# googleinterns/multimodal-long-transformer-2021

Hardware: AMD Instinct MI355X
Metric: train-step samples/sec + attention TFLOPS, 4096-tok seq (higher is better)
Workload: dtype bf16; 1 GPU; BASELINE config 3: BERT-base dims, S=4096 (2+63^2 patches+125 text), radius 64 + 8 global tokens, bf16, per-GPU batch 4; step=train_step, per_gpu_batch=4, global_batch=4, seq_len=4096, parallelism=dp1, ranks_seen=1, params=111009852, optimizer=AdamW (fused flat step, bf16 shadow weights) + polynomial lr, clip 1.0, grad_allreduce=none (1 GPU), grad_reduce=mean, step_launch=HIP graph replay (recorded after 3 eager steps)

## Files before the change

### multimodal-long-transformer-2021_amd/csrc/embed.hip

```cpp
#include "../../include/mmt_attn.h"
#include "../../include/mmt_layer.h"

#include "layer_common.h"
#include "mmt_err.h"

namespace mmt {

constexpr int kEmbedCut = 32;
constexpr int kEmbedBlocks = 1024;

struct EmbedParams {
  long rows;
  int S, H, vocab, seg_vocab, patch_start, n_patch;
  float eps, inv_keep;
  uint32_t thresh16, seed_lo, seed_hi;
  const unsigned long long* epoch;
  const int *word_ids, *seg_ids, *order, *sorted_ids;
  const float *word_table, *seg_table, *pos_table, *gamma, *beta, *patch_bias;
  const void* patch;
  void* out;
  float *mean_out, *rstd_out;
  const void* dout;
  const float *mean, *rstd;
  float* dword_table;
  float* part;
  float* pieces;
  void* dpatch;
  int nblocks;
  const int *starts, *slots;
  int n_ex, pos_rows;
  const int *image_entry, *text_entry, *prefix_ids, *text_ids, *text_len;
  int n_images, n_texts;
  int* valid_len_out;
};

struct PackedPos { int local, e, pj; bool has_patch; };
__device__ __forceinline__ PackedPos packed_pos(const EmbedParams& p, long row, int s) {
  PackedPos o;
  const int st = min(max(p.starts[row], 0), p.S - 1);
  o.local = min(max(s - st, 0), p.S - 1);
  o.e = p.slots ? p.slots[row] : -1;
  o.pj = o.local - p.patch_start;
// ... 78 lines not shown
      load_param(p.beta + c * 8, bt);
#pragma unroll
      for (int i = 0; i < 8; ++i) {
        float w = (v[j][i] - mean) * rstd * g[i] + bt[i];
        if (p.thresh16) w = layer_drop_bits16(layer_drop_row(sd.lo, sd.hi, row), (uint32_t)(c * 8 + i)) >= p.thresh16 ? w * p.inv_keep : 0.f;
        y[i] = w;
      }
      if (sg_ok) {
        load_param(p.seg_table + (long)sg * p.H + c * 8, t);
#pragma unroll
        for (int i = 0; i < 8; ++i) y[i] += t[i];
      }
      if (p.pos_table) {
        load_param(p.pos_table + (long)ps * p.H + c * 8, t);
#pragma unroll
        for (int i = 0; i < 8; ++i) y[i] += t[i];
      }
      if (has_patch) {
        Chunk<T>::load(reinterpret_cast<const T*>(p.patch) + ((long)pe * p.n_patch + pj) * p.H + c * 8, t);
#pragma unroll
        for (int i = 0; i < 8; ++i) y[i] += t[i];
        if (p.patch_bias) {
          load_param(p.patch_bias + c * 8, t);
#pragma unroll
          for (int i = 0; i < 8; ++i) y[i] += t[i];
        }
      }
      Chunk<T>::store(reinterpret_cast<T*>(p.out) + off, y);
    }
  }
}

template <typename T, int NCH, bool PK = false>
__global__ __launch_bounds__(256) void embed_bwd_kernel(const EmbedParams p) {
  const SeedPair sd = effective_seed(p.seed_lo, p.seed_hi, p.epoch);
  __shared__ float red[4][64 * NCH * 8];
  const int lane = threadIdx.x & 63, wave = threadIdx.x >> 6;
  const int nch = p.H >> 3;
  const float invH = 1.f / (float)p.H;
  float acc_g[NCH][8], acc_bt[NCH][8], gam[NCH][8];
#pragma unroll
  for (int j = 0; j < NCH; ++j) {
#pragma unroll
    for (int i = 0; i < 8; ++i) { acc_g[j][i] = 0.f; acc_bt[j][i] = 0.f; gam[j][i] = 0.f; }
    if (lane + 64 * j < nch) load_param(p.gamma + (lane + 64 * j) * 8, gam[j]);
  }
  for (long pos = (long)blockIdx.x * 4 + wave; pos < p.rows; pos += (long)gridDim.x * 4) {
    const int id = p.sorted_ids[pos];
    const bool first = pos == 0 || p.sorted_ids[pos - 1] != id;
    if (!first && (pos % kEmbedCut) != 0) continue;
    const long cut = (pos / kEmbedCut + 1) * kEmbedCut;
    const long lim = cut < p.rows ? cut : p.rows;
    const bool id_ok = (unsigned)id < (unsigned)p.vocab;
    float xw[NCH][8], acc[NCH][8];
#pragma unroll
    for (int j = 0; j < NCH; ++j) {
#pragma unroll
      for (int i = 0; i < 8; ++i) { xw[j][i] = 0.f; acc[j][i] = 0.f; }
      if (id_ok && lane + 64 * j < nch) load_param(p.word_table + (long)id * p.H + (lane + 64 * j) * 8, xw[j]);
    }
    int n_rows, rowv = 0;
    {
      const long me = pos + (lane & 31);
      const bool in_piece = me < lim && p.sorted_ids[me] == id;
      if (me < lim) rowv = p.order[me];
      const unsigned long long mism = ~__ballot(in_piece) & 0xFFFFFFFFull;
      n_rows = mism ? __builtin_ctzll(mism) : 32;
    }
    const long e = pos + n_rows;
    const int row0 = __builtin_amdgcn_readfirstlane(rowv);
    const float mean = p.mean[row0], rstd = p.rstd[row0];
    float tsum[NCH][8];
#pragma unroll
    for (int j = 0; j < NCH; ++j)
#pragma unroll
      for (int i = 0; i < 8; ++i) tsum[j][i] = 0.f;
    for (int k0 = 0; k0 < n_rows; k0 += 4) {
      float t[4][NCH][8];
      int rows4[4];
#pragma unroll
      for (int u = 0; u < 4; ++u) {
        const int k = min(k0 + u, n_rows - 1);
        rows4[u] = __builtin_amdgcn_readlane(rowv, k);
#pragma unroll
        for (int j = 0; j < NCH; ++j) {
          const int c = lane + 64 * j;
#pragma unroll
          for (int i = 0; i < 8; ++i) t[u][j][i] = 0.f;
          if (c < nch && k0 + u < n_rows) Chunk<T>::load(reinterpret_cast<const T*>(p.dout) + (long)rows4[u] * p.H + c * 8, t[u][j]);
        }
      }
#pragma unroll
// ... 22 lines not shown
          }
        }
      }
    }
    {
      float xh[NCH][8];
      float s1 = 0.f, s2 = 0.f;
#pragma unroll
      for (int j = 0; j < NCH; ++j)
#pragma unroll
        for (int i = 0; i < 8; ++i) {
          const bool live = lane + 64 * j < nch;
          xh[j][i] = live ? (xw[j][i] - mean) * rstd : 0.f;
          const float dyh = tsum[j][i] * gam[j][i];
          s1 += dyh;
          s2 += dyh * xh[j][i];
          acc_g[j][i] += tsum[j][i] * xh[j][i];
          acc_bt[j][i] += tsum[j][i];
        }
      const float c1 = wave_sum(s1) * invH, c2 = wave_sum(s2) * invH;
#pragma unroll
      for (int j = 0; j < NCH; ++j)
#pragma unroll
        for (int i = 0; i < 8; ++i) acc[j][i] = rstd * (tsum[j][i] * gam[j][i] - c1 - xh[j][i] * c2);
    }
    const bool run_ends = e >= p.rows || p.sorted_ids[e] != id;
    const bool whole = first && run_ends;
    if (!id_ok) continue;
#pragma unroll
    for (int j = 0; j < NCH; ++j) {
      const int c = lane + 64 * j;
      if (c >= nch) continue;
      if (whole) {
        float* dst = p.dword_table + (long)id * p.H + c * 8;
        float cur[8];
        load_param(dst, cur);
#pragma unroll
        for (int i = 0; i < 8; ++i) cur[i] += acc[j][i];
        Chunk<float>::store(dst, cur);
      } else {
        Chunk<float>::store(p.pieces + pos * p.H + c * 8, acc[j]);
      }
    }
  }
  int set = 0;
  auto flush = [&](float (&a)[NCH][8]) {
    __syncthreads();
#pragma unroll
    for (int j = 0; j < NCH; ++j)
#pragma unroll
      for (int i = 0; i < 8; ++i) red[wave][(lane + 64 * j) * 8 + i] = a[j][i];
    __syncthreads();
    for (int col = threadIdx.x; col < p.H; col += 256)
      p.part[((long)blockIdx.x * 2 + set) * p.H + col] = (red[0][col] + red[1][col]) + (red[2][col] + red[3][col]);
    ++set;
  };
  flush(acc_g);
  flush(acc_bt);
}

template <int NCH>
__global__ __launch_bounds__(256) void embed_bwd_runs_kernel(const EmbedParams p) {
  const int lane = threadIdx.x & 63, wave = threadIdx.x >> 6;
  const int nch = p.H >> 3;
  for (long pos = (long)blockIdx.x * 4 + wave; pos < p.rows; pos += (long)gridDim.x * 4) {
    const int id = p.sorted_ids[pos];
    const bool first = pos == 0 || p.sorted_ids[pos - 1] != id;
    const long cut = (pos / kEmbedCut + 1) * kEmbedCut;
    if (!first || cut >= p.rows || p.sorted_ids[cut] != id || (unsigned)id >= (unsigned)p.vocab) continue;
    float acc[NCH][8];
#pragma unroll
    for (int j = 0; j < NCH; ++j) {
#pragma unroll
      for (int i = 0; i < 8; ++i) acc[j][i] = 0.f;
      if (lane + 64 * j < nch) load_param(p.pieces + pos * p.H + (lane + 64 * j) * 8, acc[j]);
    }
    for (long q = cut; q < p.rows && p.sorted_ids[q] == id; q += kEmbedCut) {
#pragma unroll
      for (int j = 0; j < NCH; ++j)
        if (lane + 64 * j < nch) {
          float t[8];
          load_param(p.pieces + q * p.H + (lane + 64 * j) * 8, t);
#pragma unroll
          for (int i = 0; i < 8; ++i) acc[j][i] += t[i];
        }
    }
#pragma unroll
    for (int j = 0; j < NCH; ++j) {
      const int c = lane + 64 * j;
      if (c >= nch) continue;
      float* dst = p.dword_table + (long)id * p.H + c * 8;
      float cur[8];
      load_param(dst, cur);
#pragma unroll
      for (int i = 0; i < 8; ++i) cur[i] += acc[j][i];
      Chunk<float>::store(dst, cur);
    }
  }
// ... 87 lines not shown
int mmt_embed_fwd_pairs(const mmt_embed_desc* d, const int32_t* image_entry, const int32_t* text_entry,
                        const int32_t* prefix_ids, const int32_t* text_ids, const int32_t* text_len, int32_t n_images,
                        int32_t n_texts, const float* word_table, const float* seg_table, const float* pos_table,
                        const float* gamma, const float* beta, const void* patch_proj, const float* patch_bias,
                        void* out, int32_t* valid_len_out, void* stream) {
  if (int rc = check_embed(d)) return rc;
  if (d->dropout_p != 0.f) return mmt::fail(MMT_E_UNSUPPORTED, "mmt_embed_fwd_pairs: forward for prediction only, dropout_p must be 0");
  if (!image_entry || !text_entry || !prefix_ids || !text_ids || !text_len || !word_table || !seg_table || !gamma || !beta ||
      !out || !valid_len_out)
    return mmt::fail(MMT_E_INVALID, "mmt_embed_fwd_pairs: NULL argument");
  if ((long)d->patch_start + d->n_patch >= d->S)
    return mmt::fail(MMT_E_INVALID, "mmt_embed_fwd_pairs: the image part [0, %d) leaves no room for text in S=%d",
                     d->patch_start + d->n_patch, d->S);
  if (d->n_patch > 0 && !patch_proj) return mmt::fail(MMT_E_INVALID, "mmt_embed_fwd_pairs: n_patch > 0 but patch_proj is NULL");
  mmt::EmbedParams p; fill_embed(p, d);
  p.word_table = word_table; p.seg_table = seg_table; p.pos_table = pos_table; p.gamma = gamma; p.beta = beta;
  p.patch = d->n_patch > 0 ? patch_proj : nullptr; p.patch_bias = patch_bias; p.out = out;
  p.image_entry = image_entry; p.text_entry = text_entry; p.prefix_ids = prefix_ids; p.text_ids = text_ids;
  p.text_len = text_len; p.n_images = n_images > 0 ? n_images : 0; p.n_texts = n_texts > 0 ? n_texts : 0;
  p.valid_len_out = valid_len_out;
  const int blocks = embed_blocks(d), nchl = ((d->H >> 3) + 63) / 64;
  hipStream_t st = (hipStream_t)stream;
#define MMT_EP(T, N) hipLaunchKernelGGL((mmt::embed_fwd_kernel<T, N, false, true>), dim3(blocks), dim3(256), 0, st, p)
#define MMT_EPN(T) do { if (nchl <= 1) MMT_EP(T, 1); else if (nchl <= 2) MMT_EP(T, 2); else MMT_EP(T, 4); } while (0)
  if (d->dtype == MMT_BF16) MMT_EPN(__bf16); else MMT_EPN(float);
#undef MMT_EPN
#undef MMT_EP
  hipError_t e = hipGetLastError();
  return e == hipSuccess ? MMT_OK : mmt::fail(MMT_E_LAUNCH, "mmt_embed_fwd_pairs: %s", hipGetErrorString(e));
}

size_t mmt_embed_workspace_bytes(const mmt_embed_desc* d) {
  if (!d || d->H <= 0 || d->rows <= 0) return 0;
  return ((size_t)mmt::kEmbedBlocks * 2 * d->H + (size_t)d->rows * d->H) * sizeof(float);
}

static int embed_bwd_any(const mmt_embed_desc* d, const void* dout, const int32_t* sorted_ids, const int32_t* order,
                  const float* word_table, const float* gamma, const float* mean, const float* rstd,
                  float* dword_table, float* dgamma, float* dbeta, void* dpatch, void* ws, size_t ws_bytes,
                  const int32_t* starts, const int32_t* slots, int n_ex, void* stream) {
  if (int rc = check_embed(d)) return rc;
  if (!dout || !sorted_ids || !order || !word_table || !gamma || !mean || !rstd || !dword_table || !dgamma || !dbeta)
    return mmt::fail(MMT_E_INVALID, "mmt_embed_bwd: NULL argument");
  if (!ws || ws_bytes < mmt_embed_workspace_bytes(d)) return mmt::fail(MMT_E_WORKSPACE, "mmt_embed_bwd: workspace too small");
  mmt::EmbedParams p; fill_embed(p, d);
  p.dout = dout; p.sorted_ids = sorted_ids; p.order = order; p.word_table = word_table; p.gamma = gamma;
  p.mean = mean; p.rstd = rstd; p.dword_table = dword_table; p.dpatch = d->n_patch > 0 ? dpatch : nullptr;
  p.part = (float*)ws; p.pieces = p.part + (size_t)mmt::kEmbedBlocks * 2 * d->H;
  p.nblocks = embed_blocks(d);
  p.starts = starts; p.slots = slots; p.n_ex = n_ex;
  const int nchl = ((d->H >> 3) + 63) / 64;
  hipStream_t st = (hipStream_t)stream;
#define MMT_EB(T, N, PK) hipLaunchKernelGGL((mmt::embed_bwd_kernel<T, N, PK>), dim3(p.nblocks), dim3(256), 0, st, p)
#define MMT_EBN(T, PK) do { if (nchl <= 1) MMT_EB(T, 1, PK); else if (nchl <= 2) MMT_EB(T, 2, PK); else MMT_EB(T, 4, PK); } while (0)
  if (starts) { if (d->dtype == MMT_BF16) MMT_EBN(__bf16, true); else MMT_EBN(float, true); }
  else { if (d->dtype == MMT_BF16) MMT_EBN(__bf16, false); else MMT_EBN(float, false); }
#undef MMT_EBN
#undef MMT_EB
  hipError_t e = hipGetLastError();
  if (e != hipSuccess) return mmt::fail(MMT_E_LAUNCH, "mmt_embed_bwd: %s", hipGetErrorString(e));
  if (nchl <= 1) hipLaunchKernelGGL(mmt::embed_bwd_runs_kernel<1>, dim3(p.nblocks), dim3(256), 0, st, p);
  else if (nchl <= 2) hipLaunchKernelGGL(mmt::embed_bwd_runs_kernel<2>, dim3(p.nblocks), dim3(256), 0, st, p);
  else hipLaunchKernelGGL(mmt::embed_bwd_runs_kernel<4>, dim3(p.nblocks), dim3(256), 0, st, p);
  if ((e = hipGetLastError()) != hipSuccess) return mmt::fail(MMT_E_LAUNCH, "mmt_embed_bwd runs: %s", hipGetErrorString(e));
  e = mmt::launch_colsum_reduce(p.part, p.nblocks, 2, d->H, dgamma, dbeta, nullptr, d->accumulate, st);
  return e == hipSuccess ? MMT_OK : mmt::fail(MMT_E_LAUNCH, "mmt_embed_bwd reduce: %s", hipGetErrorString(e));
}

int mmt_embed_bwd(const mmt_embed_desc* d, const void* dout, const int32_t* sorted_ids, const int32_t* order,
                  const float* word_table, const float* gamma, const float* mean, const float* rstd,
                  float* dword_table, float* dgamma, float* dbeta, void* dpatch, void* ws, size_t ws_bytes,
                  void* stream) {
  return embed_bwd_any(d, dout, sorted_ids, order, word_table, gamma, mean, rstd, dword_table, dgamma, dbeta, dpatch, ws,
                       ws_bytes, nullptr, nullptr, 0, stream);
}

int mmt_embed_bwd_packed(const mmt_embed_desc* d, const void* dout, const int32_t* sorted_ids, const int32_t* order,
                         const float* word_table, const float* gamma, const float* mean, const float* rstd,
                         float* dword_table, float* dgamma, float* dbeta, void* dpatch,
                         const int32_t* example_starts, const int32_t* patch_slots, int32_t n_examples,
                         void* ws, size_t ws_bytes, void* stream) {
  if (!example_starts) return mmt::fail(MMT_E_INVALID, "mmt_embed_bwd_packed: example_starts is NULL");
  if (dpatch && (!patch_slots || n_examples <= 0)) return mmt::fail(MMT_E_INVALID, "mmt_embed_bwd_packed: dpatch needs patch_slots and n_examples > 0");
  return embed_bwd_any(d, dout, sorted_ids, order, word_table, gamma, mean, rstd, dword_table, dgamma, dbeta, dpatch, ws,
                       ws_bytes, example_starts, patch_slots, n_examples, stream);
}

}
```

### multimodal-long-transformer-2021_amd/csrc/fused_layer.hip

```cpp
#include "../../include/mmt_attn.h"
#include "../../include/mmt_layer.h"

#include <hip/hip_runtime.h>

#include <cmath>
#include <cstdarg>
#include <cstdio>

#include "layer_common.h"
#include <cstring>
#include "mmt_err.h"

namespace mmt {

struct LayerParams {
  long rows;
  int H;
  float eps, inv_keep;
  uint32_t thresh16, seed_lo, seed_hi;
  const unsigned long long* epoch;
  const void *a, *b, *c;
  const float *p0, *p1, *p2;
  const float *mean, *rstd;
  void *o0, *o1;
// ... 64 lines not shown
        const int c = lane + 64 * j;
        if (c < nch) ChunkW<T, W>::store(reinterpret_cast<T*>(p.o0) + row * p.H + c * W, v[j]);
      }
    }
    if (HAS_LN) {
      float s = 0.f;
#pragma unroll
      for (int j = 0; j < NCH; ++j)
#pragma unroll
        for (int i = 0; i < W; ++i) s += v[j][i];
      const float mean = wave_sum(s) * invH;
      float q = 0.f;
#pragma unroll
      for (int j = 0; j < NCH; ++j)
        if (lane + 64 * j < nch)
#pragma unroll
          for (int i = 0; i < W; ++i) { const float d = v[j][i] - mean; q += d * d; }
      const float rstd = rsqrtf(wave_sum(q) * invH + p.eps);
      if (lane == 0) { p.s0[row] = mean; p.s1[row] = rstd; }
#pragma unroll
      for (int j = 0; j < NCH; ++j) {
        const int c = lane + 64 * j;
        if (c < nch) {
          float y[W];
#pragma unroll
          for (int i = 0; i < W; ++i) y[i] = (v[j][i] - mean) * rstd * g[j][i] + bt[j][i];
          ChunkW<T, W>::store(reinterpret_cast<T*>(p.o1) + row * p.H + c * W, y);
        }
      }
    }
  }
}

template <typename T, int W, int NCH, bool RESID, bool HAS_LN>
__global__ __launch_bounds__(256, (W * NCH <= 12 ? 4 : 1)) void resid_ln_bwd_kernel(const LayerParams p) {
  const SeedPair sd = effective_seed(p.seed_lo, p.seed_hi, p.epoch);
  __shared__ float red[4][64 * NCH * W];
  const int lane = threadIdx.x & 63, wave = threadIdx.x >> 6;
  const int nch = p.H / W;
  const float invH = 1.f / (float)p.H;
  const bool has_in = p.a != nullptr;
  float acc_b[NCH][W], acc_g[NCH][W], acc_bt[NCH][W];
  float gam[NCH][W];
#pragma unroll
  for (int j = 0; j < NCH; ++j) {
#pragma unroll
    for (int i = 0; i < W; ++i) { acc_b[j][i] = 0.f; acc_g[j][i] = 0.f; acc_bt[j][i] = 0.f; gam[j][i] = 0.f; }
    if (HAS_LN && lane + 64 * j < nch) load_param_w<W>(p.p1 + (lane + 64 * j) * W, gam[j]);
  }
  for (long row = (long)blockIdx.x * 4 + wave; row < p.rows; row += (long)gridDim.x * 4) {
    RawW<T, W> ra[NCH], rb[NCH], rc[NCH];
    const uint32_t drow = layer_drop_row(sd.lo, sd.hi, row);
    float mean = 0.f, rstd = 0.f;
    if (HAS_LN) { mean = p.mean[row]; rstd = p.rstd[row]; }
#pragma unroll
    for (int j = 0; j < NCH; ++j) {
      const int ch = lane + 64 * j;
      ra[j].zero(); rb[j].zero(); rc[j].zero();
      if (ch < nch) {
        const long off = row * p.H + ch * W;
        if (has_in) ra[j].load(reinterpret_cast<const T*>(p.a) + off);
        if (HAS_LN) { rb[j].load(reinterpret_cast<const T*>(p.b) + off); rc[j].load(reinterpret_cast<const T*>(p.c) + off); }
      }
    }
    float c1 = 0.f, c2 = 0.f;
    if (HAS_LN) {
      float s1 = 0.f, s2 = 0.f;
#pragma unroll
      for (int j = 0; j < NCH; ++j)
#pragma unroll
        for (int i = 0; i < W; ++i) {
          const float dh = rb[j].get(i);
          const float xh = (rc[j].get(i) - mean) * rstd;
          const float dyh = dh * gam[j][i];
          s1 += dyh;
          s2 += dyh * xh;
          acc_g[j][i] += dh * xh;
          acc_bt[j][i] += dh;
        }
      c1 = wave_sum(s1) * invH; c2 = wave_sum(s2) * invH;
#pragma unroll
      for (int j = 0; j < NCH; ++j) { rb[j].opaque(); rc[j].opaque(); }
    }
#pragma unroll
    for (int j = 0; j < NCH; ++j) {
      const int ch = lane + 64 * j;
      if (ch < nch) {
        const long off = row * p.H + ch * W;
        float dx[W];
#pragma unroll
        for (int i = 0; i < W; ++i) {
          float g = ra[j].get(i);
          if (HAS_LN) {
            const float xh = (rc[j].get(i) - mean) * rstd;
            g += rstd * (rb[j].get(i) * gam[j][i] - c1 - xh * c2);
          }
          dx[i] = g;
        }
        if (RESID) {
          float d_o[W];
#pragma unroll
          for (int i = 0; i < W; ++i) {
            float t = dx[i];
            if (p.thresh16) t = layer_drop_bits16(drow, (uint32_t)(ch * W + i)) >= p.thresh16 ? t * p.inv_keep : 0.f;
            d_o[i] = t;
            acc_b[j][i] += t;
          }
          ChunkW<T, W>::store(reinterpret_cast<T*>(p.o0) + off, d_o);
        }
        ChunkW<T, W>::store(reinterpret_cast<T*>(p.o1) + off, dx);
      }
    }
  }
  constexpr int kSets = (RESID ? 1 : 0) + (HAS_LN ? 2 : 0);
  int set = 0;
  auto flush = [&](float (&acc)[NCH][W]) {
    __syncthreads();
#pragma unroll
    for (int j = 0; j < NCH; ++j)
#pragma unroll
      for (int i = 0; i < W; ++i) red[wave][(lane + 64 * j) * W + i] = acc[j][i];
    __syncthreads();
    for (int col = threadIdx.x; col < p.H; col += 256)
      p.part[((long)blockIdx.x * kSets + set) * p.H + col] = (red[0][col] + red[1][col]) + (red[2][col] + red[3][col]);
    ++set;
  };
  if (RESID) flush(acc_b);
  if (HAS_LN) { flush(acc_g); flush(acc_bt); }
}

constexpr int kCsCols = 16, kCsGroups = 64;
__device__ __forceinline__ void colsum_reduce_body(int blk, const float* part, int nblocks, int ksets, int H,
                                                   float* o0, float* o1, float* o2, int accumulate, float (*red)[kCsCols]) {
  const int c = threadIdx.x & (kCsCols - 1), grp = threadIdx.x / kCsCols;
  const int idx = blk * kCsCols + c;
  const int total = ksets * H;
  const int per = (nblocks + kCsGroups - 1) / kCsGroups;
  const int lo = grp * per, hi = min(nblocks, lo + per);
  float a0 = 0.f, a1 = 0.f, a2 = 0.f, a3 = 0.f;
  if (idx < total) {
    int b = lo;
    for (; b + 3 < hi; b += 4) {
      a0 += part[(long)b * total + idx];
      a1 += part[(long)(b + 1) * total + idx];
      a2 += part[(long)(b + 2) * total + idx];
      a3 += part[(long)(b + 3) * total + idx];
    }
    for (; b < hi; ++b) a0 += part[(long)b * total + idx];
  }
  red[grp][c] = (a0 + a1) + (a2 + a3);
  __syncthreads();
  if (grp == 0 && idx < total) {
    float s = 0.f;
#pragma unroll
    for (int g = 0; g < kCsGroups; ++g) s += red[g][c];
    const int set = idx / H, col = idx - set * H;
    float* dst = set == 0 ? o0 : (set == 1 ? o1 : o2);
    dst[col] = accumulate ? dst[col] + s : s;
  }
}
__global__ __launch_bounds__(1024) void colsum_reduce_kernel(const float* part, int nblocks, int ksets, int H,
                                                             float* o0, float* o1, float* o2, int accumulate) {
  __shared__ float red[kCsGroups][kCsCols];
  colsum_reduce_body(blockIdx.x, part, nblocks, ksets, H, o0, o1, o2, accumulate, red);
// ... 214 lines not shown
    p4[1] = *reinterpret_cast<const f32x4*>(prm + i1); g4[1] = *reinterpret_cast<const f32x4*>(grd + i1);
    a4[1] = *reinterpret_cast<const f32x4*>(m1 + i1); b4[1] = *reinterpret_cast<const f32x4*>(m2 + i1);
#pragma unroll
    for (int u = 0; u < 2; ++u) {
      if (u == 1 && !two) break;
      const long i = u ? i1 : i0;
      const float decay = u ? decay1 : decay0;
      f32x4 o4;
      bf16x4 s4;
#pragma unroll
      for (int j = 0; j < 4; ++j) {
        const float g = g4[u][j] * gs;
        const float mm = a.beta1 * a4[u][j] + (1.f - a.beta1) * g;
        const float vv = a.beta2 * b4[u][j] + (1.f - a.beta2) * g * g;
        const float denom = sqrtf(vv) * a.inv_sqrt_bc2 + a.eps;
        const float pn = p4[u][j] * decay - a.lr * a.inv_bc1 * (mm / denom);
        a4[u][j] = mm; b4[u][j] = vv; o4[j] = pn; s4[j] = (__bf16)pn;
      }
      *reinterpret_cast<f32x4*>(prm + i) = o4;
      *reinterpret_cast<f32x4*>(m1 + i) = a4[u];
      *reinterpret_cast<f32x4*>(m2 + i) = b4[u];
      if (shadow) *reinterpret_cast<bf16x4*>(shadow + i) = s4;
      if (a.zero_grad) *reinterpret_cast<f32x4*>(grd + i) = f32x4{0.f, 0.f, 0.f, 0.f};
    }
  }
}

}

namespace {

#define lfail mmt::fail

constexpr int kRowBlocks = 1024;
constexpr int kGeluRowSplit = 512;

int check_rows(const mmt_rows_desc* d, int max_h) {
  if (!d) return lfail(MMT_E_INVALID, "desc is NULL");
  if (d->rows <= 0 || d->H <= 0 || (d->H & 7)) return lfail(MMT_E_INVALID, "rows must be positive and H a positive multiple of 8");
  if (d->H > max_h) return lfail(MMT_E_UNSUPPORTED, "H=%d exceeds the built maximum %d", d->H, max_h);
  if (d->dtype != MMT_F32 && d->dtype != MMT_BF16) return lfail(MMT_E_INVALID, "bad dtype %d", d->dtype);
  if (!(d->dropout_p >= 0.f && d->dropout_p < 1.f)) return lfail(MMT_E_INVALID, "dropout_p must be in [0,1)");
  return MMT_OK;
}

int row_blocks_fwd(const mmt_rows_desc* d) {
  const long need = (d->rows + 3) / 4;
  return (int)(need < 1024 ? need : 1024);
}

int row_blocks(const mmt_rows_desc* d) {
  const long need = (d->rows + 3) / 4;
  return (int)(need < kRowBlocks ? need : kRowBlocks);
}

void fill(mmt::LayerParams& p, const mmt_rows_desc* d) {
  p = mmt::LayerParams{};
  p.rows = d->rows; p.H = d->H; p.eps = d->eps;
  if (d->dropout_p > 0.f) {
    p.thresh16 = mmt::dropout_thresh16(d->dropout_p);
    p.inv_keep = mmt::dropout_inv_keep(p.thresh16);
    p.seed_lo = (uint32_t)d->dropout_seed; p.seed_hi = (uint32_t)(d->dropout_seed >> 32);
    p.epoch = reinterpret_cast<const unsigned long long*>(d->dropout_epoch);
  }
}

void row_tiling(int H, int& W, int& nchl) {
  const int n8 = ((H >> 3) + 63) / 64, n4 = ((H >> 2) + 63) / 64;
  if (n4 <= 3 && n4 * 256 < n8 * 512) { W = 4; nchl = n4; }
  else { W = 8; nchl = n8 <= 2 ? n8 : (n8 <= 4 ? 4 : 8); }
}

template <bool RESID, bool HAS_LN>
hipError_t launch_fwd(const mmt::LayerParams& p, bool bf16, hipStream_t st, int blocks) {
  int W, nchl; row_tiling(p.H, W, nchl);
#define MMT_FWD(T, WW, N) hipLaunchKernelGGL((mmt::resid_ln_fwd_kernel<T, WW, N, RESID, HAS_LN>), dim3(blocks), dim3(256), 0, st, p)
#define MMT_FWD_T(T) \
  if (W == 4) { if (nchl <= 1) MMT_FWD(T, 4, 1); else if (nchl <= 2) MMT_FWD(T, 4, 2); else MMT_FWD(T, 4, 3); } \
  else { if (nchl <= 1) MMT_FWD(T, 8, 1); else if (nchl <= 2) MMT_FWD(T, 8, 2); else if (nchl <= 4) MMT_FWD(T, 8, 4); else MMT_FWD(T, 8, 8); }
  if (bf16) { MMT_FWD_T(__bf16) } else { MMT_FWD_T(float) }
#undef MMT_FWD_T
#undef MMT_FWD
  return hipGetLastError();
}

template <bool RESID, bool HAS_LN>
hipError_t launch_bwd(const mmt::LayerParams& p, bool bf16, hipStream_t st, int blocks) {
  int W, nchl; row_tiling(p.H, W, nchl);
#define MMT_BWD(T, WW, N) hipLaunchKernelGGL((mmt::resid_ln_bwd_kernel<T, WW, N, RESID, HAS_LN>), dim3(blocks), dim3(256), 0, st, p)
#define MMT_BWD_T(T) \
  if (W == 4) { if (nchl <= 1) MMT_BWD(T, 4, 1); else if (nchl <= 2) MMT_BWD(T, 4, 2); else MMT_BWD(T, 4, 3); } \
  else { if (nchl <= 1) MMT_BWD(T, 8, 1); else if (nchl <= 2) MMT_BWD(T, 8, 2); else MMT_BWD(T, 8, 4); }
  if (bf16) { MMT_BWD_T(__bf16) } else { MMT_BWD_T(float) }
#undef MMT_BWD_T
#undef MMT_BWD
  return hipGetLastError();
}

constexpr int kMaxLnH = 2048;

}

extern "C" {

size_t mmt_layer_workspace_bytes(const mmt_rows_desc* d) {
  if (!d || d->H <= 0) return 0;
  const size_t a = (size_t)kRowBlocks * 3 * d->H * sizeof(float);
  const size_t b = (size_t)kGeluRowSplit * d->H * sizeof(float);
  return a > b ? a : b;
}

int mmt_ln_fwd(const mmt_rows_desc* d, const void* x, const float* gamma, const float* beta,
               void* y, float* mean, float* rstd, void* stream) {
  if (int rc = check_rows(d, kMaxLnH)) return rc;
  if (!x || !gamma || !beta || !y || !mean || !rstd) return lfail(MMT_E_INVALID, "mmt_ln_fwd: NULL argument");
  mmt::LayerParams p; fill(p, d);
  p.b = x; p.p1 = gamma; p.p2 = beta; p.o1 = y; p.s0 = mean; p.s1 = rstd;
  hipError_t e = launch_fwd<false, true>(p, d->dtype == MMT_BF16, (hipStream_t)stream, row_blocks_fwd(d));
  return e == hipSuccess ? MMT_OK : lfail(MMT_E_LAUNCH, "mmt_ln_fwd: %s", hipGetErrorString(e));
}

int mmt_ln_bwd(const mmt_rows_desc* d, const void* dy, const void* x, const float* gamma,
               const float* mean, const float* rstd, void* dx, float* dgamma, float* dbeta,
               void* ws, size_t ws_bytes, void* stream) {
  return mmt_ln_bwd_add(d, dy, x, gamma, mean, rstd, nullptr, dx, dgamma, dbeta, ws, ws_bytes, stream);
}

int mmt_ln_bwd_add(const mmt_rows_desc* d, const void* dy, const void* x, const float* gamma,
                   const float* mean, const float* rstd, const void* dx_in, void* dx, float* dgamma, float* dbeta,
                   void* ws, size_t ws_bytes, void* stream) {
  if (int rc = check_rows(d, kMaxLnH)) return rc;
  if (!dy || !x || !gamma || !mean || !rstd || !dx || !dgamma || !dbeta) return lfail(MMT_E_INVALID, "mmt_ln_bwd: NULL argument");
  if (!ws || ws_bytes < mmt_layer_workspace_bytes(d)) return lfail(MMT_E_WORKSPACE, "mmt_ln_bwd: workspace too small");
  mmt::LayerParams p; fill(p, d);
  p.a = dx_in; p.b = dy; p.c = x; p.p1 = gamma; p.mean = mean; p.rstd = rstd; p.o1 = dx; p.part = (float*)ws;
  p.nblocks = row_blocks(d);
  hipStream_t st = (hipStream_t)stream;
  hipError_t e = launch_bwd<false, true>(p, d->dtype == MMT_BF16, st, p.nblocks);
  if (e != hipSuccess) return lfail(MMT_E_LAUNCH, "mmt_ln_bwd: %s", hipGetErrorString(e));
  if (d->defer_reduce) return MMT_OK;
  hipLaunchKernelGGL(mmt::colsum_reduce_kernel, dim3((2 * d->H + mmt::kCsCols - 1) / mmt::kCsCols), dim3(1024), 0, st, p.part, p.nblocks, 2, d->H, dgamma, dbeta, (float*)nullptr, d->accumulate);
  e = hipGetLastError();
  return e == hipSuccess ? MMT_OK : lfail(MMT_E_LAUNCH, "mmt_ln_bwd reduce: %s", hipGetErrorString(e));
}

int mmt_residual_block_fwd(const mmt_rows_desc* d, const void* o, const float* bias, const void* x,
                           const float* gamma, const float* beta, void* x_new, void* h, float* mean,
                           float* rstd, void* stream) {
  if (int rc = check_rows(d, kMaxLnH)) return rc;
  if (!o || !bias || !x || !x_new) return lfail(MMT_E_INVALID, "mmt_residual_block_fwd: NULL argument");
  if (gamma && (!beta || !h || !mean || !rstd)) return lfail(MMT_E_INVALID, "mmt_residual_block_fwd: LayerNorm outputs missing");
  mmt::LayerParams p; fill(p, d);
  p.a = o; p.b = x; p.p0 = bias; p.p1 = gamma; p.p2 = beta; p.o0 = x_new; p.o1 = h; p.s0 = mean; p.s1 = rstd;
  const bool bf16 = d->dtype == MMT_BF16;
  hipError_t e = gamma ? launch_fwd<true, true>(p, bf16, (hipStream_t)stream, row_blocks_fwd(d))
                       : launch_fwd<true, false>(p, bf16, (hipStream_t)stream, row_blocks_fwd(d));
  return e == hipSuccess ? MMT_OK : lfail(MMT_E_LAUNCH, "mmt_residual_block_fwd: %s", hipGetErrorString(e));
}

int mmt_residual_block_bwd(const mmt_rows_desc* d, const void* dx_new_in, const void* dh,
                           const void* x_new, const float* gamma, const float* mean, const float* rstd,
                           void* d_o, void* dx, float* dbias, float* dgamma, float* dbeta,
                           void* ws, size_t ws_bytes, void* stream) {
  if (int rc = check_rows(d, kMaxLnH)) return rc;
  const bool has_ln = gamma != nullptr;
  if (!d_o || !dx || !dbias) return lfail(MMT_E_INVALID, "mmt_residual_block_bwd: NULL output");
  if (has_ln && (!dh || !x_new || !mean || !rstd || !dgamma || !dbeta)) return lfail(MMT_E_INVALID, "mmt_residual_block_bwd: LayerNorm arguments missing");
  if (!has_ln && !dx_new_in) return lfail(MMT_E_INVALID, "mmt_residual_block_bwd: no incoming gradient");
  if (!ws || ws_bytes < mmt_layer_workspace_bytes(d)) return lfail(MMT_E_WORKSPACE, "mmt_residual_block_bwd: workspace too small");
  mmt::LayerParams p; fill(p, d);
  p.a = dx_new_in; p.b = dh; p.c = x_new; p.p1 = gamma; p.mean = mean; p.rstd = rstd; p.o0 = d_o; p.o1 = dx;
  p.part = (float*)ws; p.nblocks = row_blocks(d);
  hipStream_t st = (hipStream_t)stream;
  const bool bf16 = d->dtype == MMT_BF16;
  hipError_t e = has_ln ? launch_bwd<true, true>(p, bf16, st, p.nblocks) : launch_bwd<true, false>(p, bf16, st, p.nblocks);
  if (e != hipSuccess) return lfail(MMT_E_LAUNCH, "mmt_residual_block_bwd: %s", hipGetErrorString(e));
  const int ksets = has_ln ? 3 : 1;
  if (d->defer_reduce) return MMT_OK;
  hipLaunchKernelGGL(mmt::colsum_reduce_kernel, dim3((ksets * d->H + mmt::kCsCols - 1) / mmt::kCsCols), dim3(1024), 0, st, p.part, p.nblocks, ksets, d->H, dbias, dgamma, dbeta, d->accumulate);
  e = hipGetLastError();
  return e == hipSuccess ? MMT_OK : lfail(MMT_E_LAUNCH, "mmt_residual_block_bwd reduce: %s", hipGetErrorString(e));
}

int mmt_colsum_reduce(const mmt_rows_desc* d, int32_t kind, const void* ws, float* o0, float* o1, float* o2,
                      void* stream) {
  if (int rc = check_rows(d, 8192)) return rc;
  if (!ws || !o0 || kind < 0 || kind > 3) return lfail(MMT_E_INVALID, "mmt_colsum_reduce: bad argument");
  int nblocks, ksets;
  if (kind == 3) { nblocks = (int)(d->rows < kGeluRowSplit ? d->rows : kGeluRowSplit); ksets = 1; }
  else { nblocks = row_blocks(d); ksets = kind == 0 ? 2 : (kind == 1 ? 3 : 1); }
  if ((ksets >= 2 && !o1) || (ksets >= 3 && !o2)) return lfail(MMT_E_INVALID, "mmt_colsum_reduce: output missing");
  hipError_t e = mmt::launch_colsum_reduce((const float*)ws, nblocks, ksets, d->H, o0, o1, o2, d->accumulate, (hipStream_t)stream);
  return e == hipSuccess ? MMT_OK : lfail(MMT_E_LAUNCH, "mmt_colsum_reduce: %s", hipGetErrorString(e));
}

int mmt_colsum_reduce_batch(int32_t n, const mmt_colsum_item* items, void* stream) {
  if (n < 1 || n > mmt::kCsBatchMax || !items) return lfail(MMT_E_INVALID, "mmt_colsum_reduce_batch: needs 1..%d items", mmt::kCsBatchMax);
  mmt::ColsumBatch g;
  std::memset(&g, 0, sizeof(g));
  g.n = n;
  int end = 0;
  for (int i = 0; i < n; ++i) {
    const mmt_colsum_item& it = items[i];
    if (!it.workspace || !it.o0 || it.kind < 0 || it.kind > 3 || it.rows <= 0 || it.H <= 0 || (it.H & 7) || it.H > 8192)
      return lfail(MMT_E_INVALID, "mmt_colsum_reduce_batch: bad item %d", i);
    const int ksets = it.kind == 0 ? 2 : (it.kind == 1 ? 3 : 1);
    if ((ksets >= 2 && !it.o1) || (ksets >= 3 && !it.o2)) return lfail(MMT_E_INVALID, "mmt_colsum_reduce_batch: output missing in item %d", i);
    mmt_rows_desc d{}; d.rows = it.rows; d.H = it.H;
    g.part[i] = (const float*)it.workspace; g.o0[i] = it.o0; g.o1[i] = it.o1; g.o2[i] = it.o2;
    g.nblocks[i] = it.kind == 3 ? (int)(it.rows < kGeluRowSplit ? it.rows : kGeluRowSplit) : row_blocks(&d);
    g.H[i] = it.H; g.ksets[i] = (unsigned char)ksets; g.accumulate[i] = it.accumulate ? 1 : 0;
    end += (ksets * it.H + mmt::kCsCols - 1) / mmt::kCsCols;
    g.blocks_end[i] = end;
  }
  for (int i = 0; i < n; ++i)
    for (int a = 0; a < g.ksets[i]; ++a) {
      const uintptr_t lo = (uintptr_t)(a == 0 ? g.o0[i] : (a == 1 ? g.o1[i] : g.o2[i])), hi = lo + (uintptr_t)g.H[i] * sizeof(float);
      for (int j = i; j < n; ++j)
        for (int b = (j == i ? a + 1 : 0); b < g.ksets[j]; ++b) {
          const uintptr_t lo2 = (uintptr_t)(b == 0 ? g.o0[j] : (b == 1 ? g.o1[j] : g.o2[j])), hi2 = lo2 + (uintptr_t)g.H[j] * sizeof(float);
          if (lo < hi2 && lo2 < hi)
            return lfail(MMT_E_INVALID, "mmt_colsum_reduce_batch: output %d of item %d overlaps output %d of item %d", b, j, a, i);
        }
    }
  hipError_t e = mmt::launch_colsum_reduce_batch(g, (hipStream_t)stream);
  return e == hipSuccess ? MMT_OK : lfail(MMT_E_LAUNCH, "mmt_colsum_reduce_batch: %s", hipGetErrorString(e));
}

int mmt_grad_clip_scale(int32_t n_slabs, const float* const* slabs, const int64_t* sizes, float max_norm,
                        float pending_scale, float* scale_out, float* norm_out, void* workspace,
                        size_t workspace_bytes, void* stream) {
  if (n_slabs < 1 || n_slabs > mmt::kMaxNormSlabs || !slabs || !sizes || !scale_out)
    return lfail(MMT_E_INVALID, "mmt_grad_clip_scale: needs 1..%d slabs and an output", mmt::kMaxNormSlabs);
  if (!workspace || workspace_bytes < (size_t)mmt::kNormBlocks * sizeof(float))
    return lfail(MMT_E_WORKSPACE, "mmt_grad_clip_scale: workspace of %zu bytes needed", (size_t)mmt::kNormBlocks * sizeof(float));
  mmt::NormSlabs a;
  a.n = n_slabs;
  for (int i = 0; i < n_slabs; ++i) {
    if (!slabs[i] || sizes[i] <= 0 || (sizes[i] & 3) || ((uintptr_t)slabs[i] & 15))
      return lfail(MMT_E_INVALID, "mmt_grad_clip_scale: slabs must be 16-byte aligned with a multiple of 4 elements");
    a.ptr[i] = slabs[i]; a.n4[i] = sizes[i] >> 2;
  }
  hipStream_t st = (hipStream_t)stream;
// ... 97 lines not shown
```

Baseline: 269.9 samples/s.

## Restructure row-reduction backward kernels: fewer, wider blocks and contiguous per-wave ranges

```diff
diff --git a/multimodal-long-transformer-2021_amd/csrc/embed.hip b/multimodal-long-transformer-2021_amd/csrc/embed.hip
--- a/multimodal-long-transformer-2021_amd/csrc/embed.hip
+++ b/multimodal-long-transformer-2021_amd/csrc/embed.hip
@@ -8,6 +8,8 @@
 
 constexpr int kEmbedCut = 32;
 constexpr int kEmbedBlocks = 1024;
+constexpr int kEmbedBwdBlocks = 256;
+constexpr int embed_bwd_waves(int nch) { return nch <= 1 ? 16 : (nch <= 2 ? 8 : 4); }
 
 struct EmbedParams {
   long rows;
@@ -152,9 +154,10 @@
 }
 
 template <typename T, int NCH, bool PK = false>
-__global__ __launch_bounds__(256) void embed_bwd_kernel(const EmbedParams p) {
+__global__ __launch_bounds__(64 * embed_bwd_waves(NCH)) void embed_bwd_kernel(const EmbedParams p) {
+  constexpr int WAVES = embed_bwd_waves(NCH);
   const SeedPair sd = effective_seed(p.seed_lo, p.seed_hi, p.epoch);
-  __shared__ float red[4][64 * NCH * 8];
+  __shared__ float red[2][WAVES][64 * NCH * 8];
   const int lane = threadIdx.x & 63, wave = threadIdx.x >> 6;
   const int nch = p.H >> 3;
   const float invH = 1.f / (float)p.H;
@@ -165,19 +168,38 @@
     for (int i = 0; i < 8; ++i) { acc_g[j][i] = 0.f; acc_bt[j][i] = 0.f; gam[j][i] = 0.f; }
     if (lane + 64 * j < nch) load_param(p.gamma + (lane + 64 * j) * 8, gam[j]);
   }
-  for (long pos = (long)blockIdx.x * 4 + wave; pos < p.rows; pos += (long)gridDim.x * 4) {
-    const int id = p.sorted_ids[pos];
-    const bool first = pos == 0 || p.sorted_ids[pos - 1] != id;
-    if (!first && (pos % kEmbedCut) != 0) continue;
+  const long n_waves = (long)gridDim.x * WAVES, per_wave = (p.rows + n_waves - 1) / n_waves;
+  const long pos_lo = ((long)blockIdx.x * WAVES + wave) * per_wave;
+  const long pos_hi = pos_lo + per_wave < p.rows ? pos_lo + per_wave : p.rows;
+  unsigned long long heads = 0;
+  long base = pos_lo - 64;
+  int my_id = 0, my_prev = 0;
+  for (;;) {
+    if (!heads) {
+      base += 64;
+      if (base >= pos_hi) break;
+      const long me = base + lane;
+      if (me < pos_hi) { my_id = p.sorted_ids[me]; my_prev = me > 0 ? p.sorted_ids[me - 1] : ~my_id; }
+      heads = __ballot(me < pos_hi && (my_prev != my_id || (me % kEmbedCut) == 0));
+      continue;
+    }
+    const int hk = __builtin_ctzll(heads);
+    heads &= heads - 1;
+    const long pos = base + hk;
+    const int id = __builtin_amdgcn_readlane(my_id, hk);
+    const bool first = __builtin_amdgcn_readlane(my_prev, hk) != id;
     const long cut = (pos / kEmbedCut + 1) * kEmbedCut;
     const long lim = cut < p.rows ? cut : p.rows;
     const bool id_ok = (unsigned)id < (unsigned)p.vocab;
-    float xw[NCH][8], acc[NCH][8];
+    float xw[NCH][8], acc[NCH][8], cur[NCH][8];
 #pragma unroll
     for (int j = 0; j < NCH; ++j) {
 #pragma unroll
-      for (int i = 0; i < 8; ++i) { xw[j][i] = 0.f; acc[j][i] = 0.f; }
-      if (id_ok && lane + 64 * j < nch) load_param(p.word_table + (long)id * p.H + (lane + 64 * j) * 8, xw[j]);
+      for (int i = 0; i < 8; ++i) { xw[j][i] = 0.f; acc[j][i] = 0.f; cur[j][i] = 0.f; }
+      if (id_ok && lane + 64 * j < nch) {
+        load_param(p.word_table + (long)id * p.H + (lane + 64 * j) * 8, xw[j]);
+        load_param(p.dword_table + (long)id * p.H + (lane + 64 * j) * 8, cur[j]);
+      }
     }
     int n_rows, rowv = 0;
     {
@@ -266,38 +288,39 @@
       const int c = lane + 64 * j;
       if (c >= nch) continue;
       if (whole) {
-        float* dst = p.dword_table + (long)id * p.H + c * 8;
-        float cur[8];
-        load_param(dst, cur);
-#pragma unroll
-        for (int i = 0; i < 8; ++i) cur[i] += acc[j][i];
-        Chunk<float>::store(dst, cur);
+#pragma unroll
+        for (int i = 0; i < 8; ++i) cur[j][i] += acc[j][i];
+        Chunk<float>::store(p.dword_table + (long)id * p.H + c * 8, cur[j]);
       } else {
         Chunk<float>::store(p.pieces + pos * p.H + c * 8, acc[j]);
       }
     }
   }
-  int set = 0;
-  auto flush = [&](float (&a)[NCH][8]) {
-    __syncthreads();
-#pragma unroll
-    for (int j = 0; j < NCH; ++j)
-#pragma unroll
-      for (int i = 0; i < 8; ++i) red[wave][(lane + 64 * j) * 8 + i] = a[j][i];
-    __syncthreads();
-    for (int col = threadIdx.x; col < p.H; col += 256)
-      p.part[((long)blockIdx.x * 2 + set) * p.H + col] = (red[0][col] + red[1][col]) + (red[2][col] + red[3][col]);
-    ++set;
-  };
-  flush(acc_g);
-  flush(acc_bt);
+#pragma unroll
+  for (int j = 0; j < NCH; ++j)
+#pragma unroll
+    for (int i = 0; i < 8; ++i) {
+      red[0][wave][(lane + 64 * j) * 8 + i] = acc_g[j][i];
+      red[1][wave][(lane + 64 * j) * 8 + i] = acc_bt[j][i];
+    }
+  __syncthreads();
+  for (int idx = threadIdx.x; idx < 2 * p.H; idx += 64 * WAVES) {
+    const int k = idx >= p.H ? 1 : 0, col = idx - k * p.H;
+    float s = red[k][0][col];
+#pragma unroll
+    for (int w = 1; w < WAVES; ++w) s += red[k][w][col];
+    p.part[(long)blockIdx.x * 2 * p.H + idx] = s;
+  }
 }
 
 template <int NCH>
 __global__ __launch_bounds__(256) void embed_bwd_runs_kernel(const EmbedParams p) {
   const int lane = threadIdx.x & 63, wave = threadIdx.x >> 6;
   const int nch = p.H >> 3;
-  for (long pos = (long)blockIdx.x * 4 + wave; pos < p.rows; pos += (long)gridDim.x * 4) {
+  const long n_waves = (long)gridDim.x * 4, per_wave = (p.rows + n_waves - 1) / n_waves;
+  const long pos_lo = ((long)blockIdx.x * 4 + wave) * per_wave;
+  const long pos_hi = pos_lo + per_wave < p.rows ? pos_lo + per_wave : p.rows;
+  for (long pos = pos_lo; pos < pos_hi; ++pos) {
     const int id = p.sorted_ids[pos];
     const bool first = pos == 0 || p.sorted_ids[pos - 1] != id;
     const long cut = (pos / kEmbedCut + 1) * kEmbedCut;
@@ -451,7 +474,7 @@
 
 size_t mmt_embed_workspace_bytes(const mmt_embed_desc* d) {
   if (!d || d->H <= 0 || d->rows <= 0) return 0;
-  return ((size_t)mmt::kEmbedBlocks * 2 * d->H + (size_t)d->rows * d->H) * sizeof(float);
+  return ((size_t)mmt::kEmbedBwdBlocks * 2 * d->H + (size_t)d->rows * d->H) * sizeof(float);
 }
 
 static int embed_bwd_any(const mmt_embed_desc* d, const void* dout, const int32_t* sorted_ids, const int32_t* order,
@@ -465,12 +488,17 @@
   mmt::EmbedParams p; fill_embed(p, d);
   p.dout = dout; p.sorted_ids = sorted_ids; p.order = order; p.word_table = word_table; p.gamma = gamma;
   p.mean = mean; p.rstd = rstd; p.dword_table = dword_table; p.dpatch = d->n_patch > 0 ? dpatch : nullptr;
-  p.part = (float*)ws; p.pieces = p.part + (size_t)mmt::kEmbedBlocks * 2 * d->H;
-  p.nblocks = embed_blocks(d);
+  p.part = (float*)ws; p.pieces = p.part + (size_t)mmt::kEmbedBwdBlocks * 2 * d->H;
   p.starts = starts; p.slots = slots; p.n_ex = n_ex;
   const int nchl = ((d->H >> 3) + 63) / 64;
+  {
+    const int waves = mmt::embed_bwd_waves(nchl <= 1 ? 1 : (nchl <= 2 ? 2 : 4));
+    const long need = (d->rows + waves - 1) / waves;
+    p.nblocks = (int)(need < mmt::kEmbedBwdBlocks ? need : mmt::kEmbedBwdBlocks);
+  }
+  const int run_blocks = embed_blocks(d);
   hipStream_t st = (hipStream_t)stream;
-#define MMT_EB(T, N, PK) hipLaunchKernelGGL((mmt::embed_bwd_kernel<T, N, PK>), dim3(p.nblocks), dim3(256), 0, st, p)
+#define MMT_EB(T, N, PK) hipLaunchKernelGGL((mmt::embed_bwd_kernel<T, N, PK>), dim3(p.nblocks), dim3(64 * mmt::embed_bwd_waves(N)), 0, st, p)
 #define MMT_EBN(T, PK) do { if (nchl <= 1) MMT_EB(T, 1, PK); else if (nchl <= 2) MMT_EB(T, 2, PK); else MMT_EB(T, 4, PK); } while (0)
   if (starts) { if (d->dtype == MMT_BF16) MMT_EBN(__bf16, true); else MMT_EBN(float, true); }
   else { if (d->dtype == MMT_BF16) MMT_EBN(__bf16, false); else MMT_EBN(float, false); }
@@ -478,9 +506,9 @@
 #undef MMT_EB
   hipError_t e = hipGetLastError();
   if (e != hipSuccess) return mmt::fail(MMT_E_LAUNCH, "mmt_embed_bwd: %s", hipGetErrorString(e));
-  if (nchl <= 1) hipLaunchKernelGGL(mmt::embed_bwd_runs_kernel<1>, dim3(p.nblocks), dim3(256), 0, st, p);
-  else if (nchl <= 2) hipLaunchKernelGGL(mmt::embed_bwd_runs_kernel<2>, dim3(p.nblocks), dim3(256), 0, st, p);
-  else hipLaunchKernelGGL(mmt::embed_bwd_runs_kernel<4>, dim3(p.nblocks), dim3(256), 0, st, p);
+  if (nchl <= 1) hipLaunchKernelGGL(mmt::embed_bwd_runs_kernel<1>, dim3(run_blocks), dim3(256), 0, st, p);
+  else if (nchl <= 2) hipLaunchKernelGGL(mmt::embed_bwd_runs_kernel<2>, dim3(run_blocks), dim3(256), 0, st, p);
+  else hipLaunchKernelGGL(mmt::embed_bwd_runs_kernel<4>, dim3(run_blocks), dim3(256), 0, st, p);
   if ((e = hipGetLastError()) != hipSuccess) return mmt::fail(MMT_E_LAUNCH, "mmt_embed_bwd runs: %s", hipGetErrorString(e));
   e = mmt::launch_colsum_reduce(p.part, p.nblocks, 2, d->H, dgamma, dbeta, nullptr, d->accumulate, st);
   return e == hipSuccess ? MMT_OK : mmt::fail(MMT_E_LAUNCH, "mmt_embed_bwd reduce: %s", hipGetErrorString(e));
diff --git a/multimodal-long-transformer-2021_amd/csrc/fused_layer.hip b/multimodal-long-transformer-2021_amd/csrc/fused_layer.hip
--- a/multimodal-long-transformer-2021_amd/csrc/fused_layer.hip
+++ b/multimodal-long-transformer-2021_amd/csrc/fused_layer.hip
@@ -120,10 +120,18 @@
   }
 }
 
+constexpr int kBwdBlocks = 256, kBwdMinLds = 84 * 1024;
+constexpr int bwd_waves(int wn, bool resid, bool has_ln) { return (!has_ln || wn <= 12) ? 16 : (wn <= 16 ? 12 : (resid ? 4 : 8)); }
+constexpr int bwd_lds_bytes(int wn, bool resid, bool has_ln) {
+  const int need = ((resid ? 1 : 0) + (has_ln ? 2 : 0)) * bwd_waves(wn, resid, has_ln) * 64 * wn * 4;
+  return need > kBwdMinLds ? need : kBwdMinLds;
+}
+
 template <typename T, int W, int NCH, bool RESID, bool HAS_LN>
-__global__ __launch_bounds__(256, (W * NCH <= 12 ? 4 : 1)) void resid_ln_bwd_kernel(const LayerParams p) {
+__global__ __launch_bounds__(64 * bwd_waves(W * NCH, RESID, HAS_LN)) void resid_ln_bwd_kernel(const LayerParams p) {
+  constexpr int WAVES = bwd_waves(W * NCH, RESID, HAS_LN);
   const SeedPair sd = effective_seed(p.seed_lo, p.seed_hi, p.epoch);
-  __shared__ float red[4][64 * NCH * W];
+  extern __shared__ float red[];
   const int lane = threadIdx.x & 63, wave = threadIdx.x >> 6;
   const int nch = p.H / W;
   const float invH = 1.f / (float)p.H;
@@ -136,7 +144,7 @@
     for (int i = 0; i < W; ++i) { acc_b[j][i] = 0.f; acc_g[j][i] = 0.f; acc_bt[j][i] = 0.f; gam[j][i] = 0.f; }
     if (HAS_LN && lane + 64 * j < nch) load_param_w<W>(p.p1 + (lane + 64 * j) * W, gam[j]);
   }
-  for (long row = (long)blockIdx.x * 4 + wave; row < p.rows; row += (long)gridDim.x * 4) {
+  for (long row = (long)blockIdx.x * WAVES + wave; row < p.rows; row += (long)gridDim.x * WAVES) {
     RawW<T, W> ra[NCH], rb[NCH], rc[NCH];
     const uint32_t drow = layer_drop_row(sd.lo, sd.hi, row);
     float mean = 0.f, rstd = 0.f;
@@ -200,24 +208,30 @@
       }
     }
   }
-  constexpr int kSets = (RESID ? 1 : 0) + (HAS_LN ? 2 : 0);
+  constexpr int kSets = (RESID ? 1 : 0) + (HAS_LN ? 2 : 0), kRowLds = 64 * W * NCH;
   int set = 0;
-  auto flush = [&](float (&acc)[NCH][W]) {
-    __syncthreads();
+  auto park = [&](float (&acc)[NCH][W]) {
+    float* dst = red + ((long)set * WAVES + wave) * kRowLds;
 #pragma unroll
     for (int j = 0; j < NCH; ++j)
 #pragma unroll
-      for (int i = 0; i < W; ++i) red[wave][(lane + 64 * j) * W + i] = acc[j][i];
-    __syncthreads();
-    for (int col = threadIdx.x; col < p.H; col += 256)
-      p.part[((long)blockIdx.x * kSets + set) * p.H + col] = (red[0][col] + red[1][col]) + (red[2][col] + red[3][col]);
+      for (int i = 0; i < W; ++i) dst[(lane + 64 * j) * W + i] = acc[j][i];
     ++set;
   };
-  if (RESID) flush(acc_b);
-  if (HAS_LN) { flush(acc_g); flush(acc_bt); }
-}
-
-constexpr int kCsCols = 16, kCsGroups = 64;
+  if (RESID) park(acc_b);
+  if (HAS_LN) { park(acc_g); park(acc_bt); }
+  __syncthreads();
+  for (int idx = threadIdx.x; idx < kSets * p.H; idx += 64 * WAVES) {
+    const int k = idx / p.H, col = idx - k * p.H;
+    const float* src = red + (long)k * WAVES * kRowLds + col;
+    float s = src[0];
+#pragma unroll
+    for (int w = 1; w < WAVES; ++w) s += src[w * kRowLds];
+    p.part[(long)blockIdx.x * kSets * p.H + idx] = s;
+  }
+}
+
+constexpr int kCsCols = 64, kCsGroups = 16;
 __device__ __forceinline__ void colsum_reduce_body(int blk, const float* part, int nblocks, int ksets, int H,
                                                    float* o0, float* o1, float* o2, int accumulate, float (*red)[kCsCols]) {
   const int c = threadIdx.x & (kCsCols - 1), grp = threadIdx.x / kCsCols;
@@ -498,7 +512,6 @@
 
 #define lfail mmt::fail
 
-constexpr int kRowBlocks = 1024;
 constexpr int kGeluRowSplit = 512;
 
 int check_rows(const mmt_rows_desc* d, int max_h) {
@@ -513,11 +526,6 @@
 int row_blocks_fwd(const mmt_rows_desc* d) {
   const long need = (d->rows + 3) / 4;
   return (int)(need < 1024 ? need : 1024);
-}
-
-int row_blocks(const mmt_rows_desc* d) {
-  const long need = (d->rows + 3) / 4;
-  return (int)(need < kRowBlocks ? need : kRowBlocks);
 }
 
 void fill(mmt::LayerParams& p, const mmt_rows_desc* d) {
@@ -550,10 +558,26 @@
   return hipGetLastError();
 }
 
+void row_tiling_bwd(int H, int& W, int& nchl) {
+  row_tiling(H, W, nchl);
+  if (W == 8 && nchl > 2) nchl = 4;
+}
+
+int row_blocks(const mmt_rows_desc* d, int kind) {
+  int W, nchl; row_tiling_bwd(d->H, W, nchl);
+  const int waves = mmt::bwd_waves(W * nchl, kind != 0, kind != 2);
+  const long need = (d->rows + waves - 1) / waves;
+  return (int)(need < mmt::kBwdBlocks ? need : mmt::kBwdBlocks);
+}
+
 template <bool RESID, bool HAS_LN>
 hipError_t launch_bwd(const mmt::LayerParams& p, bool bf16, hipStream_t st, int blocks) {
-  int W, nchl; row_tiling(p.H, W, nchl);
-#define MMT_BWD(T, WW, N) hipLaunchKernelGGL((mmt::resid_ln_bwd_kernel<T, WW, N, RESID, HAS_LN>), dim3(blocks), dim3(256), 0, st, p)
+  int W, nchl; row_tiling_bwd(p.H, W, nchl);
+#define MMT_BWD(T, WW, N) do { \
+    constexpr int lds = mmt::bwd_lds_bytes(WW * N, RESID, HAS_LN); \
+    (void)hipFuncSetAttribute(reinterpret_cast<const void*>(mmt::resid_ln_bwd_kernel<T, WW, N, RESID, HAS_LN>), hipFuncAttributeMaxDynamicSharedMemorySize, lds); \
+    hipLaunchKernelGGL((mmt::resid_ln_bwd_kernel<T, WW, N, RESID, HAS_LN>), dim3(blocks), dim3(64 * mmt::bwd_waves(WW * N, RESID, HAS_LN)), lds, st, p); \
+  } while (0)
 #define MMT_BWD_T(T) \
   if (W == 4) { if (nchl <= 1) MMT_BWD(T, 4, 1); else if (nchl <= 2) MMT_BWD(T, 4, 2); else MMT_BWD(T, 4, 3); } \
   else { if (nchl <= 1) MMT_BWD(T, 8, 1); else if (nchl <= 2) MMT_BWD(T, 8, 2); else MMT_BWD(T, 8, 4); }
@@ -571,7 +595,7 @@
 
 size_t mmt_layer_workspace_bytes(const mmt_rows_desc* d) {
   if (!d || d->H <= 0) return 0;
-  const size_t a = (size_t)kRowBlocks * 3 * d->H * sizeof(float);
+  const size_t a = (size_t)mmt::kBwdBlocks * 3 * d->H * sizeof(float);
   const size_t b = (size_t)kGeluRowSplit * d->H * sizeof(float);
   return a > b ? a : b;
 }
@@ -600,7 +624,7 @@
   if (!ws || ws_bytes < mmt_layer_workspace_bytes(d)) return lfail(MMT_E_WORKSPACE, "mmt_ln_bwd: workspace too small");
   mmt::LayerParams p; fill(p, d);
   p.a = dx_in; p.b = dy; p.c = x; p.p1 = gamma; p.mean = mean; p.rstd = rstd; p.o1 = dx; p.part = (float*)ws;
-  p.nblocks = row_blocks(d);
+  p.nblocks = row_blocks(d, 0);
   hipStream_t st = (hipStream_t)stream;
   hipError_t e = launch_bwd<false, true>(p, d->dtype == MMT_BF16, st, p.nblocks);
   if (e != hipSuccess) return lfail(MMT_E_LAUNCH, "mmt_ln_bwd: %s", hipGetErrorString(e));
@@ -636,7 +660,7 @@
   if (!ws || ws_bytes < mmt_layer_workspace_bytes(d)) return lfail(MMT_E_WORKSPACE, "mmt_residual_block_bwd: workspace too small");
   mmt::LayerParams p; fill(p, d);
   p.a = dx_new_in; p.b = dh; p.c = x_new; p.p1 = gamma; p.mean = mean; p.rstd = rstd; p.o0 = d_o; p.o1 = dx;
-  p.part = (float*)ws; p.nblocks = row_blocks(d);
+  p.part = (float*)ws; p.nblocks = row_blocks(d, has_ln ? 1 : 2);
   hipStream_t st = (hipStream_t)stream;
   const bool bf16 = d->dtype == MMT_BF16;
   hipError_t e = has_ln ? launch_bwd<true, true>(p, bf16, st, p.nblocks) : launch_bwd<true, false>(p, bf16, st, p.nblocks);
@@ -654,7 +678,7 @@
   if (!ws || !o0 || kind < 0 || kind > 3) return lfail(MMT_E_INVALID, "mmt_colsum_reduce: bad argument");
   int nblocks, ksets;
   if (kind == 3) { nblocks = (int)(d->rows < kGeluRowSplit ? d->rows : kGeluRowSplit); ksets = 1; }
-  else { nblocks = row_blocks(d); ksets = kind == 0 ? 2 : (kind == 1 ? 3 : 1); }
+  else { nblocks = row_blocks(d, kind); ksets = kind == 0 ? 2 : (kind == 1 ? 3 : 1); }
   if ((ksets >= 2 && !o1) || (ksets >= 3 && !o2)) return lfail(MMT_E_INVALID, "mmt_colsum_reduce: output missing");
   hipError_t e = mmt::launch_colsum_reduce((const float*)ws, nblocks, ksets, d->H, o0, o1, o2, d->accumulate, (hipStream_t)stream);
   return e == hipSuccess ? MMT_OK : lfail(MMT_E_LAUNCH, "mmt_colsum_reduce: %s", hipGetErrorString(e));
@@ -674,7 +698,7 @@
     if ((ksets >= 2 && !it.o1) || (ksets >= 3 && !it.o2)) return lfail(MMT_E_INVALID, "mmt_colsum_reduce_batch: output missing in item %d", i);
     mmt_rows_desc d{}; d.rows = it.rows; d.H = it.H;
     g.part[i] = (const float*)it.workspace; g.o0[i] = it.o0; g.o1[i] = it.o1; g.o2[i] = it.o2;
-    g.nblocks[i] = it.kind == 3 ? (int)(it.rows < kGeluRowSplit ? it.rows : kGeluRowSplit) : row_blocks(&d);
+    g.nblocks[i] = it.kind == 3 ? (int)(it.rows < kGeluRowSplit ? it.rows : kGeluRowSplit) : row_blocks(&d, it.kind);
     g.H[i] = it.H; g.ksets[i] = (unsigned char)ksets; g.accumulate[i] = it.accumulate ? 1 : 0;
     end += (ksets * it.H + mmt::kCsCols - 1) / mmt::kCsCols;
     g.blocks_end[i] = end;
```

Result: no change. 272.1 samples/s, median of 6 (+0.8%).
